# aayush9400/3D-Condtional-Stable-Diffusion

Hardware: AMD Instinct MI355X
Metric: latent volumes/sec at 32^3x8ch T=1000 DDPM (higher is better)
Workload: dtype f32 (f16 hi+lo x3 MFMA, f32 accumulate)

## Files before the change

3d-condtional-stable-diffusion_amd/csrc/dm3d_conv.hip:

```cpp
#include <algorithm>
#include <cstdlib>
#include "dm3d_conv_args.h"
#include <math.h>

namespace {

template <int TD, int TH, int TW, int S, int KS, int WM, int WN>
__global__ __launch_bounds__(256, 2) void conv3d_igemm_f32(const ConvArgs p) {
    constexpr int CK = 16, LDV = CK + 4, NT = 64;
    constexpr int TM = TD * TH * TW;
    constexpr int HD = (TD - 1) * S + KS, HH = (TH - 1) * S + KS, HW = (TW - 1) * S + KS;
    constexpr int HVOX = HD * HH * HW;
    constexpr int TAPS = KS * KS * KS;
    constexpr int MR = TM / WM / 32, NR = NT / WN / 32;
    constexpr int NTHR = WM * WN * 64;
    constexpr int NSLOT = (HVOX * 4 + NTHR - 1) / NTHR;
    static_assert(NTHR == 256, "kernel assumes 4 waves");
    static_assert(TM % (WM * 32) == 0 && NT % (WN * 32) == 0, "tile split");

    extern __shared__ __attribute__((aligned(16))) float smem[];
    float* lds_in = smem;
    float* lds_w = smem + HVOX * LDV;

    const int tid = threadIdx.x;
// ... 98 lines not shown
            const bool last_tap = tap + 1 == TAPS;
            {
                int nt = tap + 1, nc = c0;
                if (last_tap) { nt = 0; nc = (ch + 1 < p.nchunks) ? c0 + CK : c0; }
                wreg = *reinterpret_cast<const f32x4*>(w_thread + (size_t)nt * w_tap_stride + nc);
            }

            const int kd = tap / (KS * KS), kh = (tap / KS) % KS, kw = tap % KS;
            const int tap_off = ((kd * HH + kh) * HW + kw) * LDV;
            const float* wbuf = lds_w + (tap & 1) * (NT * LDV);
            const float* a_lds[MR];
            const float* b_lds[NR];
#pragma unroll
            for (int mr = 0; mr < MR; ++mr) a_lds[mr] = a_base[mr] + tap_off;
#pragma unroll
            for (int nr = 0; nr < NR; ++nr) b_lds[nr] = wbuf + b_off[nr];
            dm3d_mma_step<MR, NR, CK>(acc, a_lds, b_lds, half);

            if (!last_tap) {
                *reinterpret_cast<f32x4*>(lds_w + ((tap + 1) & 1) * (NT * LDV) + w_lds_off) = wreg;
                __syncthreads();
            }
        }
    }

    const int vrow = p.vec ? (p.vec_idx ? p.vec_idx[b] : b) : 0;
    const size_t sample_elems = (size_t)p.fd * p.fh * p.fw * p.cout;
#pragma unroll
    for (int nr = 0; nr < NR; ++nr) {
        const int n = n0 + wn * (NT / WN) + nr * 32 + l32;
        const bool n_ok = n < p.cout;
        const int nc = n_ok ? n : p.cout - 1;
        float add = p.bias ? p.bias[nc] : 0.0f;
        if (p.vec) add += p.vec[(size_t)vrow * p.vec_ld + nc];
#pragma unroll
        for (int mr = 0; mr < MR; ++mr) {
            size_t o[16];
            bool ok[16];
            float rv[16];
#pragma unroll
            for (int r = 0; r < 16; ++r) {
                const int row = wm * (TM / WM) + mr * 32 + dm3d_acc_row(r, half);
                const int oz = oz0 + row / (TH * TW), oy = oy0 + (row / TW) % TH, ox = ox0 + row % TW;
                ok[r] = n_ok && oz < p.od && oy < p.oh && ox < p.ow;
                o[r] = ok[r] ? ((((size_t)b * p.fd + oz * p.os + ooz) * p.fh + oy * p.os + ooy) * p.fw + ox * p.os + oox) * p.cout + n : 0;
            }
            if (p.res) {
#pragma unroll
                for (int r = 0; r < 16; ++r) rv[r] = p.res[o[r]];
            }
#pragma unroll
            for (int r = 0; r < 16; ++r) {
                float v = acc[mr][nr][r] + add;
                if (p.relu) v = fmaxf(v, 0.0f);
                if (p.prelu) { const float al = p.prelu[o[r] % sample_elems]; v = v > 0.0f ? v : al * v; }
                if (p.res) v += rv[r];
                if (p.relu_out) v = fmaxf(v, 0.0f);
                if (ok[r]) p.out[o[r]] = v;
            }
        }
    }
}

template <int TD, int TH, int TW, int S, int KS, int WM, int WN>
int launch_conv(ConvArgs& a, hipStream_t st) {
    constexpr int LDV = 20;
    constexpr int HVOX = ((TD - 1) * S + KS) * ((TH - 1) * S + KS) * ((TW - 1) * S + KS);
    constexpr size_t lds = (size_t)(HVOX * LDV + 2 * 64 * LDV) * sizeof(float);
    a.bd = (a.od + TD - 1) / TD;
    a.bh = (a.oh + TH - 1) / TH;
    a.bw = (a.ow + TW - 1) / TW;
    static std::atomic<bool> attr_set[64] = {};
    if (int dev = dm3d_dyn_lds(lds, attr_set, "conv", &conv3d_igemm_f32<TD, TH, TW, S, KS, WM, WN>); dev < 0) return dev;
    dim3 grid((unsigned)(a.batch * a.bd * a.bh * a.bw), (unsigned)(a.coutpad / 64), a.parity ? 8u : 1u);
    hipLaunchKernelGGL((conv3d_igemm_f32<TD, TH, TW, S, KS, WM, WN>), grid, dim3(256), lds, st, a);
    return dm3d_launch_check("conv3d_igemm_f32");
}

}


struct ConvKnobs {
    bool pair_off; int ksplit_mode; long split_wgs, split_target; int split_minchunks, split_maxparts; bool wino_split_off;
    int v3_td; long wide_wgs; bool wino_off; int wino_minchunks;
};
static ConvKnobs conv_knobs() {
    auto num = [](const char* name, long dflt) { const char* e = getenv(name); return e ? atol(e) : dflt; };
    auto zero = [](const char* name) { const char* e = getenv(name); return e && e[0] == '0'; };
    static const ConvKnobs once = {
        zero("DM3D_CONV_PAIR"),
        (int)num("DM3D_CONV_KSPLIT", -1),
        num("DM3D_CONV_SPLIT_WGS", 256),
        num("DM3D_CONV_SPLIT_TARGET", 512),
        (int)num("DM3D_CONV_SPLIT_MINCHUNKS", 2),
        (int)num("DM3D_CONV_SPLIT_MAXPARTS", 16),
        zero("DM3D_CONV_WINO_SPLIT"),
        0, 0, false, 0};
    ConvKnobs k = once;
    k.v3_td = (int)num("DM3D_CONV_V3_TD", 0);
    k.wide_wgs = num("DM3D_CONV_WIDE_WGS", 512);
    k.wino_off = zero("DM3D_CONV_WINO");
    k.wino_minchunks = (int)num("DM3D_CONV_WINO_MINCHUNKS", 2);
    return k;
}

static long split_tiles(const ConvArgs& a, int td) {
    return (long)a.batch * ((a.od + td - 1) / td) * ((a.oh + 7) / 8) * ((a.ow + 7) / 8) * (a.coutpad / 64) * (a.parity ? 8 : 1);
}

static int direct_ksplit(const ConvArgs& a, const ConvKnobs& K) {
    const long wgs = split_tiles(a, 4);
    if (K.ksplit_mode == 0 || wgs > K.split_wgs || a.nchunks < 4) return 1;
    int best = 1;
    for (int d = 2; d <= K.split_maxparts; ++d) {
        if (a.nchunks % d != 0 || a.nchunks / d < K.split_minchunks) continue;
        best = d;
        if (wgs * d >= K.split_target) break;
    }
    return best;
}

static int winograd_ksplit(const ConvArgs& a, const ConvKnobs& K) {
    if (K.wino_split_off || a.nchunks % 2 != 0 || a.nchunks < 16) return 1;
    const long wgs = (long)a.batch * (a.od / 8) * (a.oh / 8) * (a.ow / 8) * (a.coutpad / 64);
    return wgs <= 128 ? 2 : 1;
}

static bool winograd_serves(const ConvArgs& a, int which, int ksplit, const ConvKnobs& K) {
    if (!a.wpk_wino || which != DM3D_CONV_K3S1 || a.parity || a.cout <= 32) return false;
    if (a.s_npairs > 0) {
        if (!a.swpk_f) return false;
        const long long svox = (long long)a.batch * a.ind * a.inh * a.inw;
        if (svox * (a.sc1 > a.sc2 ? a.sc1 : a.sc2) * 4 >= (1ll << 32)) return false;
    }
    if (a.od % 8 != 0 || a.oh % 8 != 0 || a.ow % 8 != 0 || a.padz != 1 || a.pady != 1 || a.padx != 1) return false;
    if (K.wino_off || a.nchunks < K.wino_minchunks) return false;
    const long long vox = (long long)a.batch * a.ind * a.inh * a.inw;
    if (vox * (a.c1 > a.c2 ? a.c1 : a.c2) * 4 >= (1ll << 32)) return false;
    const long wgs = (long)a.batch * (a.od / 8) * (a.oh / 8) * (a.ow / 8) * (a.coutpad / 64) * ksplit;
    const long need = K.wide_wgs;
    return wgs >= need || wgs == 256 || (ksplit > 1 && wgs >= (need < 256 ? need : 256L));
}

static int direct_td(const ConvArgs& a, const ConvKnobs& K) {
    if (K.v3_td == 4) return 4;
    if (K.v3_td != 8 && (a.parity || a.s_npairs > 0)) return 4;
    if ((a.out_h2 || a.post_scale) && a.od % 8 != 0) return 4;
    return split_tiles(a, 8) >= K.wide_wgs ? 8 : 4;
}

ConvLaunch dm3d_conv_resolve(const dm3d_conv_desc* d) {
    ConvLaunch r{};
    if (!d) return r;
    const ConvKnobs K = conv_knobs();
    ConvArgs a{};
    a.x1 = d->x1; a.x2 = d->x2; a.c1 = d->c1; a.c2 = d->c2;
    a.ind = d->in_d; a.inh = d->in_h; a.inw = d->in_w;
    const bool par_mode = d->upsample || d->transpose;
    const int cstride = (par_mode || d->stride != 2) ? 1 : 2;
    a.lgd = d->in_d; a.lgh = d->in_h; a.lgw = d->in_w;
    a.od = (d->in_d + cstride - 1) / cstride;
    a.oh = (d->in_h + cstride - 1) / cstride;
    a.ow = (d->in_w + cstride - 1) / cstride;
    a.parity = par_mode ? 1 : 0;
    a.os = par_mode ? 2 : 1;
    a.fd = a.od * a.os; a.fh = a.oh * a.os; a.fw = a.ow * a.os;
    auto pad_front = [&](int in, int out) { int t = (out - 1) * cstride + d->ksize - in; return t > 0 ? t / 2 : 0; };
    a.padz = pad_front(a.lgd, a.od); a.pady = pad_front(a.lgh, a.oh); a.padx = pad_front(a.lgw, a.ow);
    const int cin = d->c1 + d->c2;
    a.cinpad = (int)dm3d_round_up(cin, DM3D_CIN_PAD);
    a.coutpad = (int)dm3d_round_up(d->cout, DM3D_COUT_PAD);
    a.nchunks = a.cinpad / 16;
    a.wpk = d->wpk; a.bias = d->bias; a.pscale = d->pro_scale; a.pshift = d->pro_shift; a.pro_bstride = d->pro_batch_stride;
    a.vec = d->vec; a.vec_idx = d->vec_idx; a.vec_ld = d->vec_ld;
    a.relu = d->relu; a.res = d->res; a.out = d->out; a.cout = d->cout;
    a.prelu = d->prelu_alpha; a.relu_out = d->relu_out;
    a.scratch = d->scratch; a.scratch_bytes = d->scratch_bytes;
    a.split_counters = d->split_counters; a.split_counter_words = d->split_counter_words;
    a.range_flag = d->range_flag; a.range_limit = d->range_limit > 0.0f ? d->range_limit : 65504.0f;
    a.wpk_wino = d->wpk_wino;
    a.x_h2 = d->x1_fmt == DM3D_FMT_H2; a.out_h2 = d->out_fmt == DM3D_FMT_H2;
    a.post_scale = d->post_scale; a.post_shift = d->post_shift;
    if (d->skip_wpk) {
        a.sx1 = d->skip_x1; a.sx2 = d->skip_x2; a.sc1 = d->skip_c1; a.sc2 = d->skip_c2; a.swpk = d->skip_wpk;
        a.s_npairs = (int)(dm3d_round_up(d->skip_c1 + d->skip_c2, 32) / 32);
        a.swpk_f = d->skip_wpk_frag;
    }
    a.batch = d->batch;
    a.out_scale = d->precision == DM3D_PREC_H3 ? ldexpf(1.0f, -d->w_exp) : 1.0f;
    if (par_mode) a.w_parity_stride = d->precision == DM3D_PREC_H3
        ? dm3d_packed_weight_h3_bytes(8, cin, d->cout) / 2 : dm3d_packed_weight_elems(8, cin, d->cout);
    a.gn_stats = d->gn_stats;
    r.a = a;
    r.which = par_mode ? DM3D_CONV_UP
                       : (d->ksize == 1 ? DM3D_CONV_K1 : (d->ksize == 4 ? DM3D_CONV_K4S2 : (d->stride == 2 ? DM3D_CONV_K3S2 : DM3D_CONV_K3S1)));

    if (d->precision != DM3D_PREC_H3) { r.family = DM3D_CONV_FAM_F32; return r; }
    if (dm3d_conv_weight_layout(d->ksize, d->stride, d->upsample, d->transpose, d->cout) != DM3D_WL_PAIR) { r.family = DM3D_CONV_FAM_TAP; return r; }
    const bool wino_geometry = r.which == DM3D_CONV_K3S1 && a.cout > 32 && a.od % 8 == 0 && a.oh % 8 == 0 && a.ow % 8 == 0;
    const int ks_direct = direct_ksplit(a, K), ks_wino = wino_geometry ? winograd_ksplit(a, K) : 1;
    auto bytes = [&](int td, int ks) { return split_tiles(a, td) * ks * (int64_t)(td * 8 * 8 * 64) * (int64_t)sizeof(float); };
    if (winograd_serves(a, r.which, a.split_counters ? ks_wino : 1, K)) {
        r.family = DM3D_CONV_FAM_WINO; r.td = 8; r.nct = 4;
        r.ksplit = a.split_counters ? ks_wino : 1;
    } else {
        r.family = DM3D_CONV_FAM_V3;
// ... 151 lines not shown
```

3d-condtional-stable-diffusion_amd/csrc/dm3d_conv_h3_host.hip:

```cpp
#include "dm3d_conv_h3v2_parts.h"

using namespace h3v2;

int dm3d_h3v2_pre_launch(const ConvLaunch& r, H3v2Launch& L) {
    ConvArgs& k = L.k;
    k = r.a;
    k.bd = (k.od + r.td - 1) / r.td; k.bh = (k.oh + 7) / 8; k.bw = (k.ow + 7) / 8;
    k.ksplit = r.ksplit;
    auto al16 = [](const void* q) { return (reinterpret_cast<size_t>(q) & 15) == 0; };
    k.epi_vec4 = k.cout % 4 == 0 && al16(k.out) && al16(k.bias) && al16(k.res) && al16(k.prelu) && al16(k.post_scale) && al16(k.post_shift)
                 && al16(k.vec) && (k.vec == nullptr || k.vec_ld % 4 == 0);
    k.split_tile_floats = 0;
    if (r.ksplit > 1) {
        k.split_tile_floats = r.tile_floats;
        DM3D_REQUIRE(k.split_counters && k.split_counter_words >= r.need_words, "conv: a Cin-split launch of %ld tiles needs split_counters of as many zeroed words (have %d)",
                     r.tiles, k.split_counter_words);
        DM3D_REQUIRE(k.scratch && (size_t)k.scratch_bytes >= (size_t)r.need_bytes,
                     "conv: scratch of %ld bytes is too small for %d parts x %ld tiles (dm3d_conv_scratch_bytes)", k.scratch_bytes, r.ksplit, r.tiles);
        DM3D_REQUIRE((size_t)r.ksplit * r.tile_floats * sizeof(float) < (1ull << 31), "conv: %d parts overflow a tile's buffer descriptor", r.ksplit);
    }
    L.stats_after = false;
    if (k.gn_stats) {
#ifdef DM3D_EPILOGUE_SCALAR
        const bool fused = false;
#else
        const bool fused = k.od % r.td == 0 && k.oh % 8 == 0 && k.ow % 8 == 0 && k.cout % 64 == 0 && k.epi_vec4 && !k.prelu
                           && !k.out_h2 && !k.post_scale;
#endif
        if (!fused) { k.gn_stats = nullptr; L.stats_after = true; }
    }
    return DM3D_OK;
}

int dm3d_h3v2_post_launch(const ConvArgs& a, const H3v2Launch& L, hipStream_t st) {
    if (L.stats_after) return dm3d_groupnorm_partials(a.out, a.batch, (int64_t)a.fd * a.fh * a.fw, a.cout, a.gn_stats, st);
    return DM3D_OK;
}

namespace {

__global__ __launch_bounds__(256) void pack_weights_h3v2_kernel(const float* __restrict__ w, int taps, int tapsp, int cin, int cout,
                                                                int nchunks, int ntiles, float scale, const float* in_scale,
                                                                _Float16* __restrict__ out, int mode) {
    const long nrec = (long)ntiles * nchunks * tapsp * 64;
    const int npar = (mode == 1 || mode == 2) ? 8 : 1;
    for (long i0 = (long)blockIdx.x * 256 + threadIdx.x; i0 < nrec * 16 * npar; i0 += (long)gridDim.x * 256) {
        const int par = (int)(i0 / (nrec * 16));
        const long i = i0 % (nrec * 16);
        const int k = (int)(i & 15);
        const long rec = i >> 4;
        const int pos = (int)(rec % 64);
        const int tap = (int)((rec / 64) % tapsp);
        const int chunk = (int)((rec / (64L * tapsp)) % nchunks);
        const int nt = (int)(rec / (64L * tapsp * nchunks));
        const int p16 = pos & 15;
        int c = 0;
        for (int cc = 0; cc < 16; ++cc) if (pi_pos(cc) == p16) c = cc;
        const int ci = chunk * 16 + k, co = nt * 64 + (mode == 3 ? 4 * c + (pos >> 4) : (pos & ~15) + c);
        float v = 0.f;
        if (ci < cin && co < cout && tap < taps) {
            if (mode == 3) {
                const int step = tap >> 1, t = step / 5;
                const int tq = (step % 5) < 3 ? (step % 5) * 3 + (tap & 1) : ((step % 5) == 3 ? ((tap & 1) ? -1 : 2) : ((tap & 1) ? 8 : 5));
                if (tq >= 0) {
                    const float g0 = w[((long)(tq * 3 + 0) * cin + ci) * cout + co], g1 = w[((long)(tq * 3 + 1) * cin + ci) * cout + co],
                                g2 = w[((long)(tq * 3 + 2) * cin + ci) * cout + co];
                    v = t == 0 ? g0 : (t == 1 ? 0.5f * ((g0 + g2) + g1) : (t == 2 ? 0.5f * ((g0 + g2) - g1) : g2));
                }
            } else
            v = mode == 1 ? dm3d_up_weight(w, cin, cout, par, tap, ci, co)
              : mode == 2 ? dm3d_convt_weight(w, cin, cout, par, tap, ci, co) : w[((long)tap * cin + ci) * cout + co];
            if (in_scale) v *= in_scale[ci];
            v *= scale;
        }
        const _Float16 hi = (_Float16)v;
        _Float16* r = out + ((long)par * nrec + rec) * REC;
        const int sw = (pos >> 2) & 3;
        r[(((k >> 3) ^ sw) << 3) + (k & 7)] = hi;
        r[(((2 + (k >> 3)) ^ sw) << 3) + (k & 7)] = (_Float16)(v - (float)hi);
    }
}

__global__ __launch_bounds__(256) void pack_skip_h3v2_kernel(const float* __restrict__ w, int cin, int cout, int npairs, int ntiles,
                                                             float scale, _Float16* __restrict__ out) {
    const long nrec = (long)ntiles * npairs * 2 * 64;
    for (long i = (long)blockIdx.x * 256 + threadIdx.x; i < nrec * 16; i += (long)gridDim.x * 256) {
        const int k = (int)(i & 15);
        const long rec = i >> 4;
        const int pos = (int)(rec % 64);
        const int t = (int)((rec / 64) % 2);
        const int pair = (int)((rec / 128) % npairs);
        const int nt = (int)(rec / (128L * npairs));
        const int p16 = pos & 15;
        int c = 0;
        for (int cc = 0; cc < 16; ++cc) if (pi_pos(cc) == p16) c = cc;
        const int ci = (pair * 2 + t) * 16 + k, co = nt * 64 + (pos & ~15) + c;
        const float v = (ci < cin && co < cout) ? w[(long)ci * cout + co] * scale : 0.0f;
        const _Float16 hi = (_Float16)v;
        const _Float16 lo = (_Float16)(v - (float)hi);
        _Float16* r = out + rec * REC;
        const int sw = (pos >> 2) & 3;
        r[(((k >> 3) ^ sw) << 3) + (k & 7)] = hi;
        r[(((2 + (k >> 3)) ^ sw) << 3) + (k & 7)] = lo;
    }
}

__global__ __launch_bounds__(256) void pack_skip_h3f_kernel(const float* __restrict__ w, int cin, int cout, int npairs, int ntiles,
                                                            float scale, _Float16* __restrict__ out) {
    const long npieces = (long)ntiles * npairs * 4 * 2 * 64;
    for (long i = (long)blockIdx.x * 256 + threadIdx.x; i < npieces * 8; i += (long)gridDim.x * 256) {
        const int j = (int)(i & 7);
        long q = i >> 3;
        const int lane = (int)(q & 63); q >>= 6;
        const int hilo = (int)(q & 1); q >>= 1;
        const int ni = (int)(q & 3); q >>= 2;
        const int pair = (int)(q % npairs);
        const int nt = (int)(q / npairs);
        const int kg = lane >> 4;
        const int ci = (pair * 2 + (kg >> 1)) * 16 + (kg & 1) * 8 + j, co = nt * 64 + 4 * (lane & 15) + ni;
        const float v = (ci < cin && co < cout) ? w[(long)ci * cout + co] * scale : 0.0f;
        const _Float16 hi = (_Float16)v;
        out[i] = hilo ? (_Float16)(v - (float)hi) : hi;
    }
}

}

int dm3d_pack_skip_h3f(const float* keras_kernel, int cin, int cout, int w_exp, void* packed, hipStream_t st) {
    const int npairs = (int)(dm3d_round_up(cin, 32) / 32), ntiles = (int)(dm3d_round_up(cout, 64) / 64);
    hipLaunchKernelGGL(pack_skip_h3f_kernel, dim3(1024), dim3(256), 0, st, keras_kernel, cin, cout, npairs, ntiles, ldexpf(1.0f, w_exp),
                       static_cast<_Float16*>(packed));
    return dm3d_launch_check("pack_skip_h3f_kernel");
}

int64_t dm3d_h3v2_skip_image_bytes(int cin, int cout) {
    return (int64_t)(dm3d_round_up(cin, 32) / 32) * 2 * dm3d_round_up(cout, 64) * REC * (int64_t)sizeof(_Float16);
}

int dm3d_pack_skip_h3v2(const float* keras_kernel, int cin, int cout, int w_exp, void* packed, hipStream_t st) {
    const int npairs = (int)(dm3d_round_up(cin, 32) / 32), ntiles = (int)(dm3d_round_up(cout, 64) / 64);
    hipLaunchKernelGGL(pack_skip_h3v2_kernel, dim3(1024), dim3(256), 0, st, keras_kernel, cin, cout, npairs, ntiles, ldexpf(1.0f, w_exp),
                       static_cast<_Float16*>(packed));
    return dm3d_launch_check("pack_skip_h3v2_kernel");
}

int64_t dm3d_h3v2_image_bytes(int taps, int cin, int cout) {
    const int g = 4, tapsp = (taps + g - 1) / g * g;
    return (int64_t)tapsp * dm3d_round_up(cout, 64) * (dm3d_round_up(cin, 16) / 16) * REC * (int64_t)sizeof(_Float16);
}

int dm3d_pack_h3v2(const float* keras_kernel, int taps, int cin, int cout, int w_exp, const float* in_scale, void* packed, int mode,
                   hipStream_t st) {
    const int nchunks = (int)(dm3d_round_up(cin, 16) / 16), ntiles = (int)(dm3d_round_up(cout, 64) / 64);
    const int g = 4;
    hipLaunchKernelGGL(pack_weights_h3v2_kernel, dim3(4096), dim3(256), 0, st, keras_kernel, taps, (taps + g - 1) / g * g, cin, cout,
                       nchunks, ntiles, ldexpf(1.0f, w_exp), in_scale, static_cast<_Float16*>(packed), mode);
    return dm3d_launch_check("pack_weights_h3v2_kernel");
}
```

3d-condtional-stable-diffusion_amd/csrc/dm3d_conv_h3w.hip:

```cpp
#include <cstdlib>
#include "dm3d_conv_h3v2_parts.h"

using namespace h3v2;

#ifdef DM3D_CLOCK_STAMPS
__device__ unsigned long long* g_dbg_stamps_w = nullptr;
extern "C" int dm3d_debug_set_stamps_wino(void* p) { return (int)hipMemcpyToSymbol(HIP_SYMBOL(g_dbg_stamps_w), &p, sizeof(p)); }
#ifndef STAMP_MASK
#define STAMP_MASK 0xffffffffu
#endif
#define STAMP(i) do { if (((STAMP_MASK >> (i)) & 1u) && g_dbg_stamps_w && wave == 0 && __builtin_amdgcn_mbcnt_lo(~0u, 0u) == 0u && cur.ntile == 0 && cur.khalf == 0 && item / ny < 4096u) { \
    g_dbg_stamps_w[(item / ny) * 32 + (i)] = __builtin_amdgcn_s_memtime(); \
    if ((i) == 1) g_dbg_stamps_w[(item / ny) * 32 + 30] = __builtin_amdgcn_s_memrealtime(); \
    if ((i) == 28) g_dbg_stamps_w[(item / ny) * 32 + 31] = __builtin_amdgcn_s_memrealtime(); } } while (0)
#else
#define STAMP(i) do { } while (0)
#endif

namespace {

template <int N, int I = 0, class F>
__device__ __forceinline__ void static_for(F&& f) {
    if constexpr (I < N) {
        f(std::integral_constant<int, I>{});
        static_for<N, I + 1>(f);
    }
}

template <int MODE>
__global__ __launch_bounds__(256, 1) void conv3d_igemm_h3w(const ConvArgs p) {
    constexpr int TD = 8, TH = 8, TW = 8, CK = 16, NT = 64, NW = 4;
    constexpr int HD = TD + 2, HH = TH + 2, HROWS = HD * HH;
    constexpr int RREC = 17;
    constexpr int NS = 20;
    constexpr int WPAIR = 2 * NT * REC;
    constexpr int RING = 4;
    constexpr int WSLOT = WPAIR * 2 / 1024 / NW;
    constexpr int NLD = 5;
    constexpr bool pro = MODE == 1, xh2 = MODE == 2;
    constexpr int PLOADS = pro ? 4 : 0;

    extern __shared__ __attribute__((aligned(16))) _Float16 smem_w[];
    _Float16* lds_w = smem_w;
    _Float16* lds_in = smem_w + RING * WPAIR;

    const int tid = threadIdx.x;
    const int lane = tid & 63, wave = __builtin_amdgcn_readfirstlane(tid >> 6);

    const int ntiles = p.coutpad / NT;
    const unsigned ny = (unsigned)(ntiles * p.ksplit);
    const int bpv = p.bd * p.bh * p.bw;
    const int cpp = p.nchunks / p.ksplit;
    unsigned item, item_end, item_step;
    {
        const unsigned n_items = (unsigned)(p.batch * bpv) * ny, G = gridDim.x, d = blockIdx.x;
        if ((G & 7u) == 0 && (n_items & 7u) == 0) {
            const unsigned per = n_items >> 3;
            item = (d & 7u) * per + (d >> 3); item_end = (d & 7u) * per + per; item_step = G >> 3;
        } else { item = d; item_end = n_items; item_step = G; }
    }
    struct Item { int b, oz0, oy0, ox0, ntile, khalf; };
    auto decode = [&](unsigned w) {
        Item it;
        unsigned brick = w / ny;
        const unsigned by = w - brick * ny;
        it.ntile = (int)(by % (unsigned)ntiles); it.khalf = (int)(by / (unsigned)ntiles);
        it.b = (int)(brick / (unsigned)bpv);
        brick -= (unsigned)(it.b * bpv);
        it.oz0 = (int)(brick / (unsigned)(p.bh * p.bw)) * TD;
        it.oy0 = (int)((brick / (unsigned)p.bw) % (unsigned)p.bh) * TH;
        it.ox0 = (int)(brick % (unsigned)p.bw) * TW;
        it.b = __builtin_amdgcn_readfirstlane(it.b); it.oz0 = __builtin_amdgcn_readfirstlane(it.oz0); it.oy0 = __builtin_amdgcn_readfirstlane(it.oy0);
        it.ox0 = __builtin_amdgcn_readfirstlane(it.ox0); it.ntile = __builtin_amdgcn_readfirstlane(it.ntile); it.khalf = __builtin_amdgcn_readfirstlane(it.khalf);
        return it;
    };
    Item cur = decode(item);
    auto vec_row = [&](const Item& it) { return p.vec ? (p.vec_idx ? p.vec_idx[it.b] : it.b) : 0; };
    int vrow_s = vec_row(cur);
    int c_lo = cur.khalf * cpp, c_hi = c_lo + cpp;
    STAMP(0);

    int piece = 0;
    bool s_act = false;
    unsigned st_addr = 0u, a_pair[2] = {0u, 0u}, wb_hi = 0u;
    int w_voff = 0;
    constexpr int DZB = HH * RREC * REC * 2, DYB = RREC * REC * 2;
    const unsigned in_addr = (unsigned)(size_t)(__attribute__((address_space(3))) _Float16*)lds_in;
    const unsigned w_addr = (unsigned)(size_t)(__attribute__((address_space(3))) _Float16*)lds_w;
    auto lane_setup = [&]() {
        int t = tid;
        asm volatile("" : "+v"(t));
        const int ln = t & 63, half = ln >> 5, q = (ln >> 4) & 1, row = ln & 15;
        piece = t & 1;
        s_act = (t >> 1) < HROWS;
        const int srow = s_act ? (t >> 1) : HROWS - 1;
        st_addr = in_addr + (unsigned)(srow * RREC * REC + ((piece ^ ((srow % HH) & 2)) << 3)) * 2u;
        const int ay = row & 3, xq = (row >> 2) ^ (row >> 3);
        const unsigned a_base = in_addr + (unsigned)((((2 * wave) * HH + ay) * RREC + xq) * (REC * 2));
        unsigned sl[3];
#pragma unroll
        for (int dy = 0; dy < 3; ++dy) sl[dy] = (unsigned)((q ^ ((ay + dy) & 2)) << 4);
        a_pair[0] = a_base + (half ? DYB + sl[1] : sl[0]);
        a_pair[1] = a_base + 2 * DYB + sl[2] + (half ? DZB : 0);
        const int b_pos = pi_pos(row);
        wb_hi = w_addr + (unsigned)((half * NT + b_pos) * REC + ((q ^ swz(b_pos)) << 3)) * 2u;
        w_voff = wave * 1024 + ln * 16;
    };
    lane_setup();
    int sb, gv0;
    bool row_in, x_lo, x_hi;
// ... 105 lines not shown
        const float x0 = x[0], x1 = x[1];
        unsigned int a, r;
        float r0, r1;
        asm volatile("v_cvt_pk_f16_f32 %0, %4, %5\n\tv_fma_mix_f32 %2, %0, -1.0, %4 op_sel_hi:[1,0,0]\n\t"
                     "v_fma_mix_f32 %3, %0, -1.0, %5 op_sel:[1,0,0] op_sel_hi:[1,0,0]\n\tv_cvt_pk_f16_f32 %1, %2, %3"
                     : "=&v"(a), "=&v"(r), "=&v"(r0), "=&v"(r1) : "v"(x0), "v"(x1));
        if (t == 3) { o3h[xt][j] = a; o3l[xt][j] = r; } else { oh[xt][j] = a; ol[xt][j] = r; }
    };
    auto chunk_masks = [&]() {
        km[0][0] = row_in && x_lo && ok0; km[0][1] = row_in && x_lo && ok1; km[1][0] = row_in && ok0; km[1][1] = row_in && ok1;
        km[2][0] = row_in && x_hi && ok0; km[2][1] = row_in && x_hi && ok1;
    };
    auto store_record = [&](const int t, const int xt) {
        if (s_act) {
            unsigned lo_addr;
            const u32x4 dh = t == 3 ? o3h[xt] : oh[xt], dl = t == 3 ? o3l[xt] : ol[xt];
            switch (t * 4 + xt) {
#define DM3D_ST(k_) case k_: asm volatile("ds_write_b128 %1, %2 offset:%4\n\tv_xor_b32 %0, 32, %1\n\tds_write_b128 %0, %3 offset:%4" \
                                          : "=&v"(lo_addr) : "v"(st_addr), "v"(dh), "v"(dl), "n"((k_) * REC * 2) : "memory"); break;
                DM3D_ST(0) DM3D_ST(1) DM3D_ST(2) DM3D_ST(3) DM3D_ST(4) DM3D_ST(5) DM3D_ST(6) DM3D_ST(7)
                DM3D_ST(8) DM3D_ST(9) DM3D_ST(10) DM3D_ST(11) DM3D_ST(12) DM3D_ST(13) DM3D_ST(14) DM3D_ST(15)
#undef DM3D_ST
            }
        }
    };
    auto lds_barrier = [&]() {
        asm volatile("s_waitcnt lgkmcnt(0)" ::: "memory");
        __builtin_amdgcn_s_barrier();
        asm volatile("" ::: "memory");
    };

#pragma unroll
    for (int hx = 0; hx < 10; ++hx) load_voxel(c_lo, hx);
    load_chunk_params(c_lo);
#pragma unroll
    for (int t = 0; t < 4; ++t)
#pragma unroll
        for (int pi = 0; pi < 4; ++pi)
#pragma unroll
            for (int ni = 0; ni < 4; ++ni) {
                acc[t][pi][ni] = f32x4v{0.f, 0.f, 0.f, 0.f};
                asm volatile("" : "+a"(acc[t][pi][ni]));
            }
    __builtin_amdgcn_s_waitcnt(0x0F70);
    chunk_masks();
#pragma unroll
    for (int hx = 0; hx < 10; ++hx) { act_quad(hx, 0); act_quad(hx, 1); }
#pragma unroll
    for (int t = 0; t < 4; ++t) {
#pragma unroll
        for (int u = 0; u < 16; ++u) split_pair(t, u >> 2, u & 3);
#pragma unroll
        for (int xt = 0; xt < 4; ++xt) store_record(t, xt);
    }
    lds_barrier();

    h8 ah[4], al[4], bh[4], bl[4];
    auto lo_of = [](const unsigned a) { unsigned r; asm volatile("v_xor_b32 %0, 32, %1" : "=v"(r) : "v"(a)); return r; };
#define DM3D_DSR(dst, addr, off) asm volatile("ds_read_b128 %0, %1 offset:%2" : "=v"(dst) : "v"(addr), "n"(off))
    constexpr int GOFF = 4 * RREC * REC * 2, SOFF = HH * RREC * REC * 2;
    auto a_hi = [&](const int s) { return a_pair[(s % 5) >= 3]; };
    auto read_a = [&](h8 (&dst)[4], const int s, const int i, const unsigned a0) {
        const int tp = s % 5;
        switch (((s / 5) * 4 + i) * 3 + (tp < 3 ? tp : tp - 3)) {
#define DM3D_RA1(t_, i_, z_) case ((t_) * 4 + (i_)) * 3 + (z_): DM3D_DSR(dst[i_], a0, (z_) * DZB + (t_) * 4 * REC * 2 + ((i_) >> 1) * SOFF + ((i_) & 1) * GOFF); break;
#define DM3D_RA(t_, i_) DM3D_RA1(t_, i_, 0) DM3D_RA1(t_, i_, 1) DM3D_RA1(t_, i_, 2)
            DM3D_RA(0, 0) DM3D_RA(0, 1) DM3D_RA(0, 2) DM3D_RA(0, 3) DM3D_RA(1, 0) DM3D_RA(1, 1) DM3D_RA(1, 2) DM3D_RA(1, 3)
            DM3D_RA(2, 0) DM3D_RA(2, 1) DM3D_RA(2, 2) DM3D_RA(2, 3) DM3D_RA(3, 0) DM3D_RA(3, 1) DM3D_RA(3, 2) DM3D_RA(3, 3)
#undef DM3D_RA
#undef DM3D_RA1
        }
    };
    auto read_b = [&](h8 (&dst)[4], const int slot, const int i, const unsigned wa) {
        switch (slot * 4 + i) {
#define DM3D_RB(k_, i_) case (k_) * 4 + (i_): DM3D_DSR(dst[i_], wa, (k_) * WPAIR * 2 + (i_) * 16 * REC * 2); break;
            DM3D_RB(0, 0) DM3D_RB(0, 1) DM3D_RB(0, 2) DM3D_RB(0, 3) DM3D_RB(1, 0) DM3D_RB(1, 1) DM3D_RB(1, 2) DM3D_RB(1, 3)
            DM3D_RB(2, 0) DM3D_RB(2, 1) DM3D_RB(2, 2) DM3D_RB(2, 3) DM3D_RB(3, 0) DM3D_RB(3, 1) DM3D_RB(3, 2) DM3D_RB(3, 3)
#undef DM3D_RB
        }
    };
    f32x4 g_y, g_z;
    float g_x0 = 0.f, g_x1 = 0.f, g_r0 = 0.f;
    unsigned int g_a = 0u;
    auto stores_at_head = [&](int p) {
        p = (p + 60) % 60;
        if (p == 37 || p == 38 || p == 40 || p == 41 || p == 44 || p == 45) return 2;
        if (p == 39 || p == 42 || p == 46) return 4;
        return p == 58 ? 8 : 0;
    };
    auto head_stores = [&](const int p) {
        if (p == 37) store_record(0, 0); else if (p == 38) store_record(0, 1); else if (p == 39) { store_record(0, 2); store_record(0, 3); }
        else if (p == 40) store_record(1, 0); else if (p == 41) store_record(1, 1); else if (p == 42) { store_record(1, 2); store_record(1, 3); }
        else if (p == 44) store_record(2, 0); else if (p == 45) store_record(2, 1); else if (p == 46) { store_record(2, 2); store_record(2, 3); }
        else if (p == 58) {
#pragma unroll
            for (int xt = 0; xt < 4; ++xt) store_record(3, xt);
        }
    };
    auto slot_gap = [&](const int G) {
        if (G == 207) { chunk_masks(); return; }
        if (G >= 208 && G < 568) {
            const int i = (G - 208) / 18, r = (G - 208) % 18;
            const int hx = i >> 1, h = i & 1, col = hx == 0 ? 0 : (hx == 9 ? 2 : 1);
            if (xh2) {
                auto mix = [&](const int c) {
                    float d;
                    const float hv = va[hx][0][c >> 1], lv = va[hx][1][c >> 1];
                    if (c & 1) asm volatile("v_fma_mix_f32 %0, %1, 1.0, %2 op_sel:[1,0,1] op_sel_hi:[1,0,1]" : "=v"(d) : "v"(hv), "v"(lv));
                    else asm volatile("v_fma_mix_f32 %0, %1, 1.0, %2 op_sel:[0,0,0] op_sel_hi:[1,0,1]" : "=v"(d) : "v"(hv), "v"(lv));
                    return d;
                };
                if (h == 0) {
                    if (r < 2) { g_y[2 * r] = mix(2 * r); g_y[2 * r + 1] = mix(2 * r + 1); }
                } else {
                    if (r < 2) {
                        const float v0 = mix(4 + 2 * r), v1 = mix(5 + 2 * r);
                        va[hx][1][2 * r] = v0; va[hx][1][2 * r + 1] = v1;
                    } else if (r < 4) {
                        const int c = 2 * (r - 2);
                        float v0 = km[col][0] ? g_y[c] : 0.0f, v1 = km[col][0] ? g_y[c + 1] : 0.0f;
                        DM3D_PIN(v0); DM3D_PIN(v1);
                        va[hx][0][c] = v0; va[hx][0][c + 1] = v1;
                    } else if (r < 6) {
                        const int c = 2 * (r - 4);
                        float v0 = km[col][0] ? va[hx][1][c] : 0.0f, v1 = km[col][0] ? va[hx][1][c + 1] : 0.0f;
                        DM3D_PIN(v0); DM3D_PIN(v1);
                        va[hx][1][c] = v0; va[hx][1][c + 1] = v1;
                    }
                }
                return;
            }
            if (!pro) {
                if (r < 2) {
                    const int c = 2 * r;
                    float v0 = km[col][h] ? va[hx][h][c] : 0.0f, v1 = km[col][h] ? va[hx][h][c + 1] : 0.0f;
                    DM3D_PIN(v0); DM3D_PIN(v1);
                    va[hx][h][c] = v0; va[hx][h][c + 1] = v1;
                }
                return;
            }
            const f32x4 sc = h ? sc1 : sc0, sh = h ? sh1 : sh0;
            if (r < 2) {
                const int c = 2 * r;
                g_y[c] = fmaf(va[hx][h][c], sc[c], sh[c]); g_y[c + 1] = fmaf(va[hx][h][c + 1], sc[c + 1], sh[c + 1]);
                DM3D_PIN(g_y[c]); DM3D_PIN(g_y[c + 1]);
            } else if (r < 4) {
                const int c = 2 * (r - 2);
                g_z[c] = g_y[c] * -1.4426950408889634f; g_z[c + 1] = g_y[c + 1] * -1.4426950408889634f;
                DM3D_PIN(g_z[c]); DM3D_PIN(g_z[c + 1]);
            } else if (r < 8) {
                g_z[r - 4] = __builtin_amdgcn_exp2f(g_z[r - 4]);
                DM3D_PIN(g_z[r - 4]);
            } else if (r < 10) {
                const int c = 2 * (r - 8);
                g_z[c] = 1.0f + g_z[c]; g_z[c + 1] = 1.0f + g_z[c + 1];
                DM3D_PIN(g_z[c]); DM3D_PIN(g_z[c + 1]);
            } else if (r < 14) {
                g_z[r - 10] = __builtin_amdgcn_rcpf(g_z[r - 10]);
                DM3D_PIN(g_z[r - 10]);
            } else if (r < 16) {
                const int c = 2 * (r - 14);
                g_y[c] = g_y[c] * g_z[c]; g_y[c + 1] = g_y[c + 1] * g_z[c + 1];
                DM3D_PIN(g_y[c]); DM3D_PIN(g_y[c + 1]);
            } else {
                const int c = 2 * (r - 16);
                float v0 = km[col][h] ? g_y[c] : 0.0f, v1 = km[col][h] ? g_y[c + 1] : 0.0f;
                DM3D_PIN(v0); DM3D_PIN(v1);
                va[hx][h][c] = v0; va[hx][h][c + 1] = v1;
            }
            return;
        }
        if ((G >= 576 && G < 672) || (G >= 688 && G < 736) || (G >= 880 && G < 928)) {
            const int t = G < 624 ? 0 : (G < 672 ? 1 : (G < 736 ? 2 : 3));
            const int q = G - (t == 0 ? 576 : (t == 1 ? 624 : (t == 2 ? 688 : 880)));
            const int u = q / 3, st = q % 3, xt = u >> 2, j = u & 3, h = j >> 1, c = 2 * (j & 1);
            if (st == 0) {
                auto d = [&](const int k, const int e) { return va[2 * xt + k][h][c + e]; };
                g_x0 = t == 0 ? d(0, 0) - d(2, 0) : (t == 1 ? d(1, 0) + d(2, 0) : (t == 2 ? d(2, 0) - d(1, 0) : d(1, 0) - d(3, 0)));
                g_x1 = t == 0 ? d(0, 1) - d(2, 1) : (t == 1 ? d(1, 1) + d(2, 1) : (t == 2 ? d(2, 1) - d(1, 1) : d(1, 1) - d(3, 1)));
                DM3D_PIN(g_x0); DM3D_PIN(g_x1);
            } else if (st == 1) {
                asm volatile("v_cvt_pk_f16_f32 %0, %2, %3\n\tv_fma_mix_f32 %1, %0, -1.0, %2 op_sel_hi:[1,0,0]" : "=&v"(g_a), "=&v"(g_r0) : "v"(g_x0), "v"(g_x1));
            } else {
                unsigned int r;
                float r1;
                asm volatile("v_fma_mix_f32 %1, %2, -1.0, %3 op_sel:[1,0,0] op_sel_hi:[1,0,0]\n\tv_cvt_pk_f16_f32 %0, %4, %1" : "=&v"(r), "=&v"(r1) : "v"(g_a), "v"(g_x1), "v"(g_r0));
                if (t == 3) { o3h[xt][j] = g_a; o3l[xt][j] = r; } else { oh[xt][j] = g_a; ol[xt][j] = r; }
            }
        }
    };
#define DM3D_MFMA(T, PI, NI, A, B) asm volatile("v_mfma_f32_16x16x32_f16 %0, %1, %2, %0" : "+a"(acc[T][PI][NI]) : "v"(A[PI]), "v"(B[NI]))
#define DM3D_WAIT_LGKM(n) asm volatile("s_waitcnt lgkmcnt(%0)" :: "n"(n) : "memory")

    bool has_next = item + item_step < item_end;
    for (;;) {
    lane_setup();
    {
        const unsigned a_lo0 = lo_of(a_hi(0));
        read_a(al, 0, 0, a_lo0); read_a(al, 0, 1, a_lo0); read_a(al, 0, 2, a_lo0); read_a(al, 0, 3, a_lo0);
    }
    read_b(bh, 0, 0, wb_hi); read_b(bh, 0, 1, wb_hi); read_b(bh, 0, 2, wb_hi); read_b(bh, 0, 3, wb_hi);
    read_a(ah, 0, 0, a_hi(0)); read_a(ah, 0, 1, a_hi(0)); read_a(ah, 0, 2, a_hi(0)); read_a(ah, 0, 3, a_hi(0));
    STAMP(1);

    for (int ch = c_lo; ch < c_hi; ++ch) {
        asm volatile("" : "+v"(gv0));
        int ch_next;
        if (ch + 1 < c_hi) { ch_next = ch + 1; w_nxt = w_cur + NS * WPAIR * 2; }
        else if (has_next) {
            const Item n = decode(item + item_step);
            stage_setup(n); ch_next = n.khalf * cpp; w_nxt = w_chunk(n.ntile, ch_next);
        }
        else { ch_next = ch; w_nxt = w_cur; }
        static_for<NS>([&](auto S_) {
            constexpr int s = decltype(S_)::value, sn = (s + 1) % NS;
            constexpr int t = s / 5, ws = s & (RING - 1), ws1 = (s + 1) & (RING - 1);
            {
                constexpr int n_out = 4;
                switch (stores_at_head(3 * s - 1)) {
                case 0: DM3D_WAIT_LGKM(n_out); break;
                case 2: DM3D_WAIT_LGKM(n_out + 2); break;
                case 4: DM3D_WAIT_LGKM(n_out + 4); break;
                default: DM3D_WAIT_LGKM(n_out + 8); break;
                }
            }
            head_stores(3 * s);
            __builtin_amdgcn_sched_barrier(0);
            unsigned b_lo = 0u, a_lo = 0u;
#pragma unroll
            for (int g = 0; g < 16; ++g) {
                DM3D_MFMA(t, g >> 2, g & 3, al, bh);
                slot_gap(16 * (3 * s) + g);
                if (g == 2) b_lo = lo_of(wb_hi);
                if (g == 3) { read_b(bl, ws, 0, b_lo); read_b(bl, ws, 1, b_lo); }
                if (g == 6) a_lo = lo_of(a_hi(sn));
                if (g == 7) { read_b(bl, ws, 2, b_lo); read_b(bl, ws, 3, b_lo); read_a(al, sn, 0, a_lo); }
                if (g == 11) { read_a(al, sn, 1, a_lo); read_a(al, sn, 2, a_lo); }
                if (g == 15) read_a(al, sn, 3, a_lo);
                __builtin_amdgcn_sched_barrier(0);
            }
            {
                constexpr int DMA_BEHIND = 2 * WSLOT;
                const int extra = halo_ops(s - 3) + halo_ops(s - 2) + halo_ops(s - 1);
#define DM3D_WAIT_VM_LGKM4(n) __builtin_amdgcn_s_waitcnt((((n) & 15) | (7 << 4) | (4 << 8) | ((((n) >> 4) & 3) << 14)))
                switch (extra) {
                case 0:  DM3D_WAIT_VM_LGKM4(DMA_BEHIND); break;
                case 4:  DM3D_WAIT_VM_LGKM4(DMA_BEHIND + 4); break;
                case 8:  DM3D_WAIT_VM_LGKM4(DMA_BEHIND + 8); break;
                case 12: DM3D_WAIT_VM_LGKM4(DMA_BEHIND + 12); break;
                case 16: DM3D_WAIT_VM_LGKM4(DMA_BEHIND + 16); break;
                default: DM3D_WAIT_VM_LGKM4(0); break;
                }
#undef DM3D_WAIT_VM_LGKM4
                __builtin_amdgcn_s_barrier();
                asm volatile("" ::: "memory");
            }
            __builtin_amdgcn_sched_barrier(0);
            const unsigned w_src = s + RING < NS ? w_cur + (s + RING) * (WPAIR * 2) : w_nxt + (s + RING - NS) * (WPAIR * 2);
            fetch_w1(w_src, ws, 0);
            head_stores(3 * s + 1);
            __builtin_amdgcn_sched_barrier(0);
#pragma unroll
            for (int g = 0; g < 16; ++g) {
                DM3D_MFMA(t, g & 3, g >> 2, ah, bh);
                slot_gap(16 * (3 * s + 1) + g);
                if ((g & 3) == 3) read_b(bh, ws1, g >> 2, wb_hi);
                if (g == 1) fetch_w1(w_src, ws, 1);
                if (s < NLD && g == 5) load_voxel(ch_next, 2 * s);
                if (s < NLD && g == 9) load_voxel(ch_next, 2 * s + 1);
                if (s == 0 && g == 13) load_chunk_params(ch_next);
                __builtin_amdgcn_sched_barrier(0);
            }
            head_stores(3 * s + 2);
            __builtin_amdgcn_sched_barrier(0);
#pragma unroll
            for (int g = 0; g < 16; ++g) {
                DM3D_MFMA(t, g >> 2, g & 3, ah, bl);
                slot_gap(16 * (3 * s + 2) + g);
                if ((g & 3) == 3) read_a(ah, sn, g >> 2, a_hi(sn));
                __builtin_amdgcn_sched_barrier(0);
            }
        });
        w_cur = w_nxt;
    }
#undef DM3D_MFMA
#undef DM3D_WAIT_LGKM
#undef DM3D_PIN
#undef DM3D_DSR
    STAMP(28);
    const Brick br = {cur.b, cur.oz0, cur.oy0, cur.ox0, p.ooz, p.ooy, p.oox, cur.ntile, cur.khalf};
    {
        asm volatile("s_waitcnt lgkmcnt(0)" ::: "memory");
        STAMP(20);
        const bool skip = p.s_npairs > 0;
        if (skip) {
#pragma unroll
            for (int pi = 0; pi < 4; ++pi)
#pragma unroll
                for (int ni = 0; ni < 4; ++ni) {
                    const f32x4v m0 = acc[0][pi][ni], m1 = acc[1][pi][ni], m2 = acc[2][pi][ni], m3 = acc[3][pi][ni];
                    acc[0][pi][ni] = (m0 + m1) + m2;
                    acc[1][pi][ni] = (m1 - m2) - m3;
                    asm volatile("" : "+a"(acc[0][pi][ni]), "+a"(acc[1][pi][ni]));
                }
            const int p_lo = p.s_npairs * cur.khalf / p.ksplit, np = p.s_npairs * (cur.khalf + 1) / p.ksplit;
            int lane_t = lane;
            asm volatile("" : "+v"(lane_t));
            const int kq = lane_t >> 4, lhalf = kq >> 1, cq = (kq & 1) * 8, row_t = lane_t & 15;
            unsigned sv[8];
#pragma unroll
            for (int t = 0; t < 8; ++t) {
                const int z = 2 * wave + (t >> 2), y = 4 * ((t >> 1) & 1) + (row_t & 3), x = 2 * ((row_t >> 2) ^ (row_t >> 3)) + (t & 1);
                sv[t] = (unsigned)(((cur.b * p.ind + cur.oz0 + z) * p.inh + cur.oy0 + y) * p.inw + cur.ox0 + x);
            }
            const char* swf = reinterpret_cast<const char*>(p.swpk_f) + (size_t)cur.ntile * p.s_npairs * 8192 + lane_t * 16;
            f32x4 ar0[2][8], ar1[2][8];
            h8 bw[2][8];
            float lim0[2], lim1[2];
            auto t_load = [&](auto SET, int pp) {
                constexpr int S = decltype(SET)::value;
                const int c0 = (pp * 2 + lhalf) * CK;
                const float* src;
                int ldc, cb;
                if (c0 < p.sc1) { src = p.sx1; ldc = p.sc1; cb = c0; } else { src = p.sx2; ldc = p.sc2; cb = c0 - p.sc1; }
                const int cpos = cb + cq;
                const bool real = src != nullptr && cb < ldc && pp < np;
                const bool k0 = real && cpos < ldc, k1 = real && cpos + 4 < ldc;
                lim0[S] = k0 ? 65504.0f : 0.0f;
                lim1[S] = k1 ? 65504.0f : 0.0f;
                const char* base = reinterpret_cast<const char*>(real ? src : p.sx1);
                const unsigned ld4 = (unsigned)(real ? ldc : p.sc1) * 4u, o0 = (unsigned)(k0 ? cpos : 0) * 4u, o1 = (unsigned)(k1 ? cpos + 4 : 0) * 4u;
#pragma unroll
                for (int t = 0; t < 8; ++t) {
                    ar0[S][t] = *reinterpret_cast<const f32x4*>(base + (sv[t] * ld4 + o0));
                    ar1[S][t] = *reinterpret_cast<const f32x4*>(base + (sv[t] * ld4 + o1));
                }
                const char* ws = swf + (size_t)(pp < p.s_npairs ? pp : p.s_npairs - 1) * 8192;
#pragma unroll
                for (int f = 0; f < 8; ++f) bw[S][f] = *reinterpret_cast<const h8*>(ws + f * 1024);
            };
#define DM3D_TMFMA(ACC, A, B) asm volatile("v_mfma_f32_16x16x32_f16 %0, %1, %2, %0" : "+a"(ACC) : "v"(A), "v"(B))
            auto t_step = [&](auto SET) {
                constexpr int S = decltype(SET)::value;
                h8 ahi[8], alo[8];
#pragma unroll
                for (int t = 0; t < 8; ++t) split8(ar0[S][t], ar1[S][t], lim0[S], lim1[S], ahi[t], alo[t]);
                __builtin_amdgcn_sched_barrier(0);
                asm volatile("s_nop 1" ::: "memory");
                __builtin_amdgcn_sched_barrier(0);
#pragma unroll
                for (int t = 0; t < 8; ++t)
#pragma unroll
                    for (int ni = 0; ni < 4; ++ni) DM3D_TMFMA(acc[t & 1][t >> 1][ni], alo[t], bw[S][2 * ni]);
#pragma unroll
                for (int t = 0; t < 8; ++t)
#pragma unroll
                    for (int ni = 0; ni < 4; ++ni) DM3D_TMFMA(acc[t & 1][t >> 1][ni], ahi[t], bw[S][2 * ni + 1]);
#pragma unroll
                for (int t = 0; t < 8; ++t)
#pragma unroll
                    for (int ni = 0; ni < 4; ++ni) DM3D_TMFMA(acc[t & 1][t >> 1][ni], ahi[t], bw[S][2 * ni]);
            };
#undef DM3D_TMFMA
// ... 128 lines not shown
```

Before: 2.271.

## Fold padded Winograd tap pair into one step, dropping a redundant MFMA pass

In the mode-3 weight packing, the padded tap slot (step%5==3) now duplicates tap 2 for both halves and zeroes the lo part of the odd half. The h3w kernel can then skip the third hi/lo MFMA pass for those steps, which cuts the pass count from 3*NS to 3*NS-NS/5. The pass schedule (store heads, slot_gap indices) is renumbered to match. Fragment roles for A hi/lo now swap between steps, and address arithmetic is done in inline asm. A knob for the Winograd split min-chunks is also added, with its default unchanged. The risk is schedule or accuracy breakage, since the lo contribution is dropped for the folded tap.

```diff
diff --git a/3d-condtional-stable-diffusion_amd/csrc/dm3d_conv.hip b/3d-condtional-stable-diffusion_amd/csrc/dm3d_conv.hip
--- a/3d-condtional-stable-diffusion_amd/csrc/dm3d_conv.hip
+++ b/3d-condtional-stable-diffusion_amd/csrc/dm3d_conv.hip
@@ -204,7 +204,7 @@
 
 struct ConvKnobs {
     bool pair_off; int ksplit_mode; long split_wgs, split_target; int split_minchunks, split_maxparts; bool wino_split_off;
-    int v3_td; long wide_wgs; bool wino_off; int wino_minchunks;
+    int v3_td; long wide_wgs; bool wino_off; int wino_minchunks, wino_split_minchunks;
 };
 static ConvKnobs conv_knobs() {
     auto num = [](const char* name, long dflt) { const char* e = getenv(name); return e ? atol(e) : dflt; };
@@ -217,12 +217,13 @@
         (int)num("DM3D_CONV_SPLIT_MINCHUNKS", 2),
         (int)num("DM3D_CONV_SPLIT_MAXPARTS", 16),
         zero("DM3D_CONV_WINO_SPLIT"),
-        0, 0, false, 0};
+        0, 0, false, 0, 0};
     ConvKnobs k = once;
     k.v3_td = (int)num("DM3D_CONV_V3_TD", 0);
     k.wide_wgs = num("DM3D_CONV_WIDE_WGS", 512);
     k.wino_off = zero("DM3D_CONV_WINO");
     k.wino_minchunks = (int)num("DM3D_CONV_WINO_MINCHUNKS", 2);
+    k.wino_split_minchunks = (int)num("DM3D_CONV_WINO_SPLIT_MINCHUNKS", 16);
     return k;
 }
 
@@ -243,7 +244,7 @@
 }
 
 static int winograd_ksplit(const ConvArgs& a, const ConvKnobs& K) {
-    if (K.wino_split_off || a.nchunks % 2 != 0 || a.nchunks < 16) return 1;
+    if (K.wino_split_off || a.nchunks % 2 != 0 || a.nchunks < K.wino_split_minchunks) return 1;
     const long wgs = (long)a.batch * (a.od / 8) * (a.oh / 8) * (a.ow / 8) * (a.coutpad / 64);
     return wgs <= 128 ? 2 : 1;
 }
diff --git a/3d-condtional-stable-diffusion_amd/csrc/dm3d_conv_h3_host.hip b/3d-condtional-stable-diffusion_amd/csrc/dm3d_conv_h3_host.hip
--- a/3d-condtional-stable-diffusion_amd/csrc/dm3d_conv_h3_host.hip
+++ b/3d-condtional-stable-diffusion_amd/csrc/dm3d_conv_h3_host.hip
@@ -58,11 +58,13 @@
         for (int cc = 0; cc < 16; ++cc) if (pi_pos(cc) == p16) c = cc;
         const int ci = chunk * 16 + k, co = nt * 64 + (mode == 3 ? 4 * c + (pos >> 4) : (pos & ~15) + c);
         float v = 0.f;
+        bool fold = false;
         if (ci < cin && co < cout && tap < taps) {
             if (mode == 3) {
                 const int step = tap >> 1, t = step / 5;
-                const int tq = (step % 5) < 3 ? (step % 5) * 3 + (tap & 1) : ((step % 5) == 3 ? ((tap & 1) ? -1 : 2) : ((tap & 1) ? 8 : 5));
-                if (tq >= 0) {
+                const int tq = (step % 5) < 3 ? (step % 5) * 3 + (tap & 1) : ((step % 5) == 3 ? 2 : ((tap & 1) ? 8 : 5));
+                fold = (step % 5) == 3 && (tap & 1);
+                {
                     const float g0 = w[((long)(tq * 3 + 0) * cin + ci) * cout + co], g1 = w[((long)(tq * 3 + 1) * cin + ci) * cout + co],
                                 g2 = w[((long)(tq * 3 + 2) * cin + ci) * cout + co];
                     v = t == 0 ? g0 : (t == 1 ? 0.5f * ((g0 + g2) + g1) : (t == 2 ? 0.5f * ((g0 + g2) - g1) : g2));
@@ -77,7 +79,7 @@
         _Float16* r = out + ((long)par * nrec + rec) * REC;
         const int sw = (pos >> 2) & 3;
         r[(((k >> 3) ^ sw) << 3) + (k & 7)] = hi;
-        r[(((2 + (k >> 3)) ^ sw) << 3) + (k & 7)] = (_Float16)(v - (float)hi);
+        r[(((2 + (k >> 3)) ^ sw) << 3) + (k & 7)] = fold ? (_Float16)0.0f : (_Float16)(v - (float)hi);
     }
 }
 
diff --git a/3d-condtional-stable-diffusion_amd/csrc/dm3d_conv_h3w.hip b/3d-condtional-stable-diffusion_amd/csrc/dm3d_conv_h3w.hip
--- a/3d-condtional-stable-diffusion_amd/csrc/dm3d_conv_h3w.hip
+++ b/3d-condtional-stable-diffusion_amd/csrc/dm3d_conv_h3w.hip
@@ -26,6 +26,8 @@
         static_for<N, I + 1>(f);
     }
 }
+
+constexpr int pass_of(int s) { return 3 * s - (s + 1) / 5; }
 
 template <int MODE>
 __global__ __launch_bounds__(256, 1) void conv3d_igemm_h3w(const ConvArgs p) {
@@ -297,25 +299,26 @@
     f32x4 g_y, g_z;
     float g_x0 = 0.f, g_x1 = 0.f, g_r0 = 0.f;
     unsigned int g_a = 0u;
+    constexpr int NPASS = 3 * NS - NS / 5;
     auto stores_at_head = [&](int p) {
-        p = (p + 60) % 60;
-        if (p == 37 || p == 38 || p == 40 || p == 41 || p == 44 || p == 45) return 2;
-        if (p == 39 || p == 42 || p == 46) return 4;
-        return p == 58 ? 8 : 0;
+        p = (p + NPASS) % NPASS;
+        if (p == 36 || p == 37 || p == 39 || p == 40 || p == 42 || p == 43) return 2;
+        if (p == 38 || p == 41 || p == 44) return 4;
+        return p == 54 ? 8 : 0;
     };
     auto head_stores = [&](const int p) {
-        if (p == 37) store_record(0, 0); else if (p == 38) store_record(0, 1); else if (p == 39) { store_record(0, 2); store_record(0, 3); }
-        else if (p == 40) store_record(1, 0); else if (p == 41) store_record(1, 1); else if (p == 42) { store_record(1, 2); store_record(1, 3); }
-        else if (p == 44) store_record(2, 0); else if (p == 45) store_record(2, 1); else if (p == 46) { store_record(2, 2); store_record(2, 3); }
-        else if (p == 58) {
+        if (p == 36) store_record(0, 0); else if (p == 37) store_record(0, 1); else if (p == 38) { store_record(0, 2); store_record(0, 3); }
+        else if (p == 39) store_record(1, 0); else if (p == 40) store_record(1, 1); else if (p == 41) { store_record(1, 2); store_record(1, 3); }
+        else if (p == 42) store_record(2, 0); else if (p == 43) store_record(2, 1); else if (p == 44) { store_record(2, 2); store_record(2, 3); }
+        else if (p == 54) {
 #pragma unroll
             for (int xt = 0; xt < 4; ++xt) store_record(3, xt);
         }
     };
     auto slot_gap = [&](const int G) {
-        if (G == 207) { chunk_masks(); return; }
-        if (G >= 208 && G < 568) {
-            const int i = (G - 208) / 18, r = (G - 208) % 18;
+        if (G == 191) { chunk_masks(); return; }
+        if (G >= 192 && G < 552) {
+            const int i = (G - 192) / 18, r = (G - 192) % 18;
             const int hx = i >> 1, h = i & 1, col = hx == 0 ? 0 : (hx == 9 ? 2 : 1);
             if (xh2) {
                 auto mix = [&](const int c) {
@@ -385,9 +388,9 @@
             }
             return;
         }
-        if ((G >= 576 && G < 672) || (G >= 688 && G < 736) || (G >= 880 && G < 928)) {
-            const int t = G < 624 ? 0 : (G < 672 ? 1 : (G < 736 ? 2 : 3));
-            const int q = G - (t == 0 ? 576 : (t == 1 ? 624 : (t == 2 ? 688 : 880)));
+        if ((G >= 560 && G < 704) || (G >= 816 && G < 864)) {
+            const int t = G < 608 ? 0 : (G < 656 ? 1 : (G < 704 ? 2 : 3));
+            const int q = G - (t == 0 ? 560 : (t == 1 ? 608 : (t == 2 ? 656 : 816)));
             const int u = q / 3, st = q % 3, xt = u >> 2, j = u & 3, h = j >> 1, c = 2 * (j & 1);
             if (st == 0) {
                 auto d = [&](const int k, const int e) { return va[2 * xt + k][h][c + e]; };
@@ -430,28 +433,39 @@
         static_for<NS>([&](auto S_) {
             constexpr int s = decltype(S_)::value, sn = (s + 1) % NS;
             constexpr int t = s / 5, ws = s & (RING - 1), ws1 = (s + 1) & (RING - 1);
+            constexpr bool pad = s % 5 == 3, pre_pad = s % 5 == 2, post_pad = s % 5 == 4;
+            constexpr int E = pass_of(s);
+            constexpr bool swapped = (((s + 1) / 5) & 1) != 0;
+            h8 (&fh)[4] = swapped ? al : ah;
+            h8 (&fl)[4] = swapped ? ah : al;
+            h8 (&fl_n)[4] = pad ? fh : fl;
+            h8 (&fh_n)[4] = pad ? fl : fh;
             {
-                constexpr int n_out = 4;
-                switch (stores_at_head(3 * s - 1)) {
+                constexpr int n_out = pad ? 0 : 4;
+                switch (post_pad ? 0 : stores_at_head(E - 1)) {
                 case 0: DM3D_WAIT_LGKM(n_out); break;
                 case 2: DM3D_WAIT_LGKM(n_out + 2); break;
                 case 4: DM3D_WAIT_LGKM(n_out + 4); break;
                 default: DM3D_WAIT_LGKM(n_out + 8); break;
                 }
             }
-            head_stores(3 * s);
+            head_stores(E);
             __builtin_amdgcn_sched_barrier(0);
             unsigned b_lo = 0u, a_lo = 0u;
 #pragma unroll
             for (int g = 0; g < 16; ++g) {
-                DM3D_MFMA(t, g >> 2, g & 3, al, bh);
-                slot_gap(16 * (3 * s) + g);
+                DM3D_MFMA(t, g >> 2, g & 3, fl, bh);
+                slot_gap(16 * E + g);
                 if (g == 2) b_lo = lo_of(wb_hi);
                 if (g == 3) { read_b(bl, ws, 0, b_lo); read_b(bl, ws, 1, b_lo); }
-                if (g == 6) a_lo = lo_of(a_hi(sn));
-                if (g == 7) { read_b(bl, ws, 2, b_lo); read_b(bl, ws, 3, b_lo); read_a(al, sn, 0, a_lo); }
-                if (g == 11) { read_a(al, sn, 1, a_lo); read_a(al, sn, 2, a_lo); }
-                if (g == 15) read_a(al, sn, 3, a_lo);
+                if (pre_pad) {
+                    if (g == 4) asm volatile("v_subrev_u32 %0, %2, %1" : "=v"(a_lo) : "v"(a_pair[1]), "n"(DZB));
+                    if (g == 5) asm volatile("v_xor_b32 %0, 32, %0" : "+v"(a_lo));
+                    if (g == 6) asm volatile("v_cndmask_b32_e64 %0, %1, %0, %2" : "+v"(a_lo) : "v"(a_pair[1]), "s"(0xffffffff00000000ull));
+                } else if (g == 6) a_lo = lo_of(a_hi(sn));
+                if (g == 7) { read_b(bl, ws, 2, b_lo); read_b(bl, ws, 3, b_lo); read_a(fl_n, sn, 0, a_lo); }
+                if (g == 11) { read_a(fl_n, sn, 1, a_lo); read_a(fl_n, sn, 2, a_lo); }
+                if (g == 15) read_a(fl_n, sn, 3, a_lo);
                 __builtin_amdgcn_sched_barrier(0);
             }
             {
@@ -473,27 +487,38 @@
             __builtin_amdgcn_sched_barrier(0);
             const unsigned w_src = s + RING < NS ? w_cur + (s + RING) * (WPAIR * 2) : w_nxt + (s + RING - NS) * (WPAIR * 2);
             fetch_w1(w_src, ws, 0);
-            head_stores(3 * s + 1);
+            head_stores(E + 1);
             __builtin_amdgcn_sched_barrier(0);
 #pragma unroll
             for (int g = 0; g < 16; ++g) {
-                DM3D_MFMA(t, g & 3, g >> 2, ah, bh);
-                slot_gap(16 * (3 * s + 1) + g);
-                if ((g & 3) == 3) read_b(bh, ws1, g >> 2, wb_hi);
+                if (pad) {
+                    DM3D_MFMA(t, g >> 2, g & 3, fl, bl);
+                    slot_gap(16 * (E + 1) + g);
+                    if (g == 2) { read_b(bh, ws1, 0, wb_hi); read_b(bh, ws1, 1, wb_hi); }
+                    if (g == 3) { read_b(bh, ws1, 2, wb_hi); read_b(bh, ws1, 3, wb_hi); }
+                    if (g == 4) read_a(fh_n, sn, 0, a_hi(sn));
+                    if (g == 7 || g == 11 || g == 15) read_a(fh_n, sn, g >> 2, a_hi(sn));
+                } else {
+                    DM3D_MFMA(t, g & 3, g >> 2, fh, bh);
+                    slot_gap(16 * (E + 1) + g);
+                    if ((g & 3) == 3) read_b(bh, ws1, g >> 2, wb_hi);
+                }
                 if (g == 1) fetch_w1(w_src, ws, 1);
                 if (s < NLD && g == 5) load_voxel(ch_next, 2 * s);
                 if (s < NLD && g == 9) load_voxel(ch_next, 2 * s + 1);
                 if (s == 0 && g == 13) load_chunk_params(ch_next);
                 __builtin_amdgcn_sched_barrier(0);
             }
-            head_stores(3 * s + 2);
-            __builtin_amdgcn_sched_barrier(0);
-#pragma unroll
-            for (int g = 0; g < 16; ++g) {
-                DM3D_MFMA(t, g >> 2, g & 3, ah, bl);
-                slot_gap(16 * (3 * s + 2) + g);
-                if ((g & 3) == 3) read_a(ah, sn, g >> 2, a_hi(sn));
+            if constexpr (!pad) {
+                head_stores(E + 2);
                 __builtin_amdgcn_sched_barrier(0);
+#pragma unroll
+                for (int g = 0; g < 16; ++g) {
+                    DM3D_MFMA(t, g >> 2, g & 3, fh, bl);
+                    slot_gap(16 * (E + 2) + g);
+                    if (!pre_pad && (g & 3) == 3) read_a(fh, sn, g >> 2, a_hi(sn));
+                    __builtin_amdgcn_sched_barrier(0);
+                }
             }
         });
         w_cur = w_nxt;
```

After: 2.325 (median of 6 runs). 2.4% higher.
